# neeek2303/EMOPortraits

Hardware: AMD Instinct MI355X
Metric: reenactment frames/sec @512x512, 1-src->N-driver (higher is better)
Workload: dtype f32

## Files before the change

emoportraits_amd/csrc/conv_igemm_f16x2_ct2.h:

```cpp
#pragma once
#include "conv_igemm_bf16x3.h"
#include "conv_split_pair_common.h"

#ifndef EMO_CT2_RES_EARLY
#define EMO_CT2_RES_EARLY 0
#endif

template <int TR, int TW, bool UPS>
struct ConvCfgS2 : ConvCfgS<TR, TW, UPS, 2> {
  using Base = ConvCfgS<TR, TW, UPS, 2>;
  static_assert(Base::NWB == 2 && Base::EPI_IN_W, "two whole weight stages in LDS; the epilogue transposes through one of them");
  static constexpr int OFF_BIAS2_F = Base::OFF_EPI_F;
  static constexpr int OFF_STAT2_F = OFF_BIAS2_F + Base::BM;
  static constexpr int LDS_BYTES = (OFF_STAT2_F + 2 * Base::WGP * Base::BM) * 4;
  static_assert(LDS_BYTES <= 160 * 1024, "LDS");
  static_assert(Base::PBUF * 16 >= 8 * 1024, "the dead weight pieces of an item's last step are dumped into a patch buffer");
};

template <int TR, int TW, bool UPS>
__global__ __launch_bounds__(256) __attribute__((amdgpu_waves_per_eu(1, 1)))
void conv_igemm_bf16x3_ct2_kernel(const ConvArgs a) {
  using Cfg = ConvCfgS2<TR, TW, UPS>;
  using opx8 = halfx8;
  constexpr int SPLIT = 2, NPL = 2, NPROD = 3;
  constexpr int BM = Cfg::BM, TM = Cfg::TM, TP = Cfg::TP, WGP = Cfg::WGP, KC = Cfg::KC;
  constexpr int PR = Cfg::PR, NQ = Cfg::NQ, NQ1 = Cfg::NQ1, SUB = Cfg::SUB, CHS = Cfg::CHS, QPG = Cfg::QPG;
  constexpr int NHQ = Cfg::NHQ, TWS = Cfg::TWS, WPLANE = Cfg::WPLANE, WROW = Cfg::WROW, PPL = Cfg::PPL, PBUF = Cfg::PBUF;

  extern __shared__ __attribute__((aligned(16))) float smem[];

  const int tid = threadIdx.x;
  const int lane = tid & 63;
  const int wave = __builtin_amdgcn_readfirstlane(tid >> 6);
  const int half = lane >> 5, l32 = lane & 31;
  const int wp = wave;
  const int p0 = wp * TP * 32;
  float sat_m = 0.0f;

  const int HW = a.H * a.W;
  const long DHW = (long)a.D * HW;
  const bool has_affine = a.scale != nullptr;
  const int epi_mode = __builtin_amdgcn_readfirstlane(a.res == nullptr ? 0 : (a.res_ups ? 2 : 1));
  const float in_scale = a.in_scale;
  const int padD = a.KD >> 1;
  constexpr float CLAMP_HI = 65504.0f;
  const float clamp_lo = a.relu_in ? 0.0f : -CLAMP_HI;
  const int nst = a.n_cchunks * a.KD;
  const int nptiles = a.tiles_x * a.tiles_y * a.tiles_z;

  const int q_u = tid % QPG;
  const int q_g = __builtin_amdgcn_readfirstlane(tid / QPG);
  const bool is_quad = q_u < PR * NQ;
  const int hq = q_u - PR * NQ;
  const bool is_halo = !is_quad && hq < NHQ;
  const int h_side = hq & 1;
  const int q_r = is_quad ? q_u / NQ : (is_halo ? hq >> 1 : 0);
  const int q_c = is_quad ? q_u - q_r * NQ : 0;
  int q_slb[4];
#pragma unroll
  for (int i = 0; i < 4; ++i) {
    const int dump = q_g * CHS + i * SUB + PR * NQ1 + (q_u & 3);
    const int own = is_quad ? q_g * CHS + i * SUB + q_r * NQ1 + q_c : q_g * CHS + h_side * SUB + q_r * NQ1 + NQ;
    q_slb[i] = ((is_quad || (is_halo && i == (h_side ? 0 : 3))) ? own : dump) * 16;
  }

  floatx16 acc_lo[2][TM][TP], acc_hi[2][TM][TP];

  const int q8 = a.n_work >> 3, r8 = a.n_work & 7;
  const int xcd = blockIdx.x & 7;
  const int n_mine = q8 + (xcd < r8 ? 1 : 0);
  const int l_base = xcd < r8 ? xcd * (q8 + 1) : r8 * (q8 + 1) + (xcd - r8) * q8;
  const int l_stride = (gridDim.x + 7) >> 3;
  int it_cotile = 0, it_n = 0, it_ptile = 0, it_x0 = 0, it_y0 = 0, it_z0 = 0;
  unsigned lq_off = 0;
  bool lq_ok = false;
  int lq_z0 = 0;
#define EMO_T_WPTR(c_, k_) (reinterpret_cast<const char*>(a.wpk) + (long)((c_) * nst + (k_)) * (3 * Cfg::WROW_BYTES))

  const int a_off = (half * BM + l32) * 16;
  EMO_P_DECLARE_B_OFF()

  const char* const lds_c = reinterpret_cast<const char*>(smem);
  char* const lds_w = reinterpret_cast<char*>(smem);
  opx8 fa_[2][NPL][TM], fb_[2][NPL][TP];
#define EMO_T_LOAD_FRAGS_PLANE(set_, pl_, wbase_, pbyte_, r_, s_)                                      \
  {                                                                                                   \
    _Pragma("unroll") for (int i = 0; i < TM; ++i)                                                    \
      fa_[set_][pl_][i] = *reinterpret_cast<const opx8*>(lds_c + a_off + ((wbase_) + (pl_) * WPLANE + (s_) * 2 * BM + i * 32) * 16); \
    _Pragma("unroll") for (int j = 0; j < TP; ++j)                                                    \
      fb_[set_][pl_][j] = *reinterpret_cast<const opx8*>(lds_c + (EMO_P_B_OFF(j, r_, s_) + (pbyte_)) + ((pl_) * PPL) * 16); \
  }

  float* const sct = smem + Cfg::OFF_SCT * 4;
  const unsigned smem_lds = (unsigned)(size_t)(__attribute__((address_space(3))) char*)reinterpret_cast<char*>(smem);
  const unsigned lane16 = (unsigned)lane * 16u;

  floatx4 qv[8];
  float q_lo, q_hi;
  int q_tix;
  floatx4 q_sc, q_sh;
  opx8 cv_h, cv_m;
  emo_intx4 xrs = emo_raw_buffer(a.x);
  unsigned usoff[8];
#pragma unroll
  for (int u = 0; u < 8; ++u) usoff[u] = (unsigned)__builtin_amdgcn_readfirstlane((int)((unsigned)u * (unsigned)DHW * 4u * (EMO_CT2_X_CONST ? 0u : 1u)));

  int n_ci0, n_zu;
  bool n_zv;
  int ld_stage, ld_cc, ld_kd;
#define EMO_T_SET_STAGE_VARS()                                                                        \
  {                                                                                                   \
    n_ci0 = ld_cc * KC;                                                                               \
    n_zu = lq_z0 + ld_kd - padD;                                                                      \
    n_zv = (unsigned)n_zu < (unsigned)a.D;                                                            \
  }
  unsigned q_vo;
#define EMO_T_ISSUE_BEGIN()                                                                           \
  {                                                                                                   \
    const int c0_ = n_ci0 + q_g * 8;                                                                  \
    const bool cv_ = c0_ < a.Cin;                                                                     \
    const int cs_ = cv_ ? c0_ : 0;                                                                    \
    const bool keep_ = lq_ok && cv_ && n_zv;                                                          \
    q_lo = keep_ ? clamp_lo : 0.0f;                                                                   \
    q_hi = keep_ ? CLAMP_HI : 0.0f;                                                                   \
    q_vo = lq_off + (EMO_CT2_X_CONST ? 0u : ((unsigned)cs_ * (unsigned)DHW + (unsigned)((n_zv ? n_zu : 0) * HW)) * 4u);   \
    q_tix = (has_affine ? cs_ : (cs_ & (Cfg::SCT - 1))) >> 2;                                         \
  }
#define EMO_T_ISSUE_LOADS(u0_, u1_)                                                                   \
  { _Pragma("unroll") for (int u = (u0_); u < (u1_); u += 2) emo_bload4x2_pinned(xrs, q_vo, usoff[u], usoff[u + 1], qv[u], qv[u + 1]); }
#define EMO_T_HALF_TABLE(hf_)                                                                         \
  {                                                                                                   \
    const floatx4* t4_ = reinterpret_cast<const floatx4*>(sct) + q_tix + (hf_);                       \
    q_sc = t4_[0]; q_sh = t4_[Cfg::SCT / 4];                                                          \
  }
#define EMO_T_TOUCH_QUAD() { _Pragma("unroll") for (int u = 0; u < 8; ++u) emo_touch4(qv[u]); }
#define EMO_T_CONV_HALF(pbyte_, i_, hf_)                                                              \
  {                                                                                                   \
    float t_[4];                                                                                      \
    _Pragma("unroll") for (int k = 0; k < 4; ++k)                                                     \
      t_[k] = __fmaf_rn(qv[4 * (hf_) + k][i_], q_sc[k], q_sh[k]);                                     \
    sat_m = __builtin_fmaxf(__builtin_fmaxf(sat_m, __builtin_fabsf(t_[0])), __builtin_fabsf(t_[1])); \
    sat_m = __builtin_fmaxf(__builtin_fmaxf(sat_m, __builtin_fabsf(t_[2])), __builtin_fabsf(t_[3])); \
    _Pragma("unroll") for (int k = 0; k < 4; k += 2)                                                  \
      emo_split_f16x2_pair(__builtin_amdgcn_fmed3f(t_[k], q_lo, q_hi), __builtin_amdgcn_fmed3f(t_[k + 1], q_lo, q_hi), \
                           cv_h, cv_m, 4 * (hf_) + k);                                                \
    if ((hf_) == 1) {                                                                                 \
      char* d_ = lds_w + (q_slb[i_] + (pbyte_));                                                      \
      *reinterpret_cast<opx8*>(d_) = cv_h;                                                            \
      *reinterpret_cast<opx8*>(d_ + PPL * 16) = cv_m;                                                 \
    }                                                                                                 \
  }
#define EMO_T_WSRC(p_) (EMO_CT2_W_CONST ? reinterpret_cast<const char*>(a.wpk) : (p_))
#define EMO_T_DMA_PIECE(ptr_, wb_, k_)                                                                \
  {                                                                                                   \
    const int row_ = (k_) / 3, j_ = wave + 4 * ((k_) % 3);                                            \
    emo_dma16_pinned_s(EMO_T_WSRC((ptr_) + (row_ * Cfg::WROW_BYTES + j_ * 1024)), lane16,             \
                       smem_lds + (unsigned)((Cfg::OFF_W + (wb_) * Cfg::WSTAGE) * 16 + row_ * Cfg::WROW_BYTES + j_ * 1024)); \
  }

  constexpr int PA3[3] = {1, 0, 0}, PB3[3] = {0, 1, 0};
  constexpr int NTE = Cfg::SCT / 256;
  float te_sc[NTE], te_sh[NTE], te_b = 0.0f;

  bool chained_in = false;
  int pp = 0;
  for (int idx8 = blockIdx.x >> 3; idx8 < n_mine; idx8 += l_stride) {
#if EMO_S_TIMING
  unsigned long long tstamp[12];
  for (int k = 0; k < 12; ++k) tstamp[k] = 0;
#endif
  EMO_S_STAMP(0)
  EMO_P_DECODE(it_, l_base + idx8)
  int nx_cotile = 0, nx_n = 0, nx_ptile = 0, nx_x0 = 0, nx_y0 = 0, nx_z0 = 0;
  bool chain_out = false, nxq_ok = false;
  unsigned nxq_off = 0;
  if (EMO_S_CHAIN && idx8 + l_stride < n_mine) {
    EMO_P_DECODE(nx_, l_base + idx8 + l_stride)
    chain_out = nx_n == it_n && nst >= 2;
    EMO_P_CURSOR_OF(nx_, nxq_ok, nxq_off)
  }
  (void)nx_ptile;
#pragma unroll
  for (int st_ = 0; st_ < 2; ++st_)
#pragma unroll
    for (int pl = 0; pl < NPL; ++pl) {
#pragma unroll
      for (int i = 0; i < TM; ++i) asm volatile("" : "=v"(fa_[st_][pl][i]));
#pragma unroll
      for (int j = 0; j < TP; ++j) asm volatile("" : "=v"(fb_[st_][pl][j]));
    }
  asm volatile("" : "=v"(cv_h));
  asm volatile("" : "=v"(cv_m));
  if (EMO_S_CHAIN && chained_in) {
    xrs = emo_raw_buffer(a.x + (long)it_n * a.Cin * DHW);
    if (tid < 2 * BM) {
      const int t2_ = tid & (BM - 1);
      smem[(tid < BM ? Cfg::OFF_BIAS_F : Cfg::OFF_BIAS2_F) + (t2_ >> 5) * 32 + (t2_ & 3) * 8 + ((t2_ & 31) >> 2)] = te_b;
    }
    const char* const w1_ = EMO_T_WPTR(it_cotile + 1, 0);
    EMO_T_DMA_PIECE(w1_, 1, 0)
    EMO_T_DMA_PIECE(w1_, 1, 1)
    EMO_P_BARRIER(2);
  } else {
#pragma unroll
    for (int u = 0; u < 8; ++u) asm volatile("" : "=v"(qv[u]));
    xrs = emo_raw_buffer(a.x + (long)it_n * a.Cin * DHW);
    EMO_P_CURSOR_OF(it_, lq_ok, lq_off)
    lq_z0 = it_z0;
#pragma unroll
    for (int k = 0; k < NTE; ++k) {
      const int c = tid + 256 * k;
      const bool real = has_affine && c < a.Cin;
      te_sc[k] = real ? a.scale[(long)it_n * a.Cin + c] : 1.0f;
      te_sh[k] = real ? a.shift[(long)it_n * a.Cin + c] : 0.0f;
    }
    if (tid < 2 * BM && a.bias != nullptr) {
      const int co_ = it_cotile * BM + tid;
      te_b = a.bias[co_ < a.Cout ? co_ : a.Cout - 1];
    }
    {
      const char* const w0_ = EMO_T_WPTR(it_cotile, 0);
#pragma unroll
      for (int k = 0; k < 9; ++k) EMO_T_DMA_PIECE(w0_, 0, k)
    }
    ld_stage = 0; ld_cc = 0; ld_kd = 0;
    EMO_T_SET_STAGE_VARS()
    EMO_T_ISSUE_BEGIN()
    EMO_T_ISSUE_LOADS(0, 8)
#pragma unroll
    for (int k = 0; k < NTE; ++k) {
      const int c = tid + 256 * k;
      if (c < min(a.Cin, Cfg::SCT)) {
        sct[c] = te_sc[k] * in_scale;
        sct[Cfg::SCT + c] = te_sh[k] * in_scale;
      }
    }
    if (tid < 2 * BM) {
      const int t2_ = tid & (BM - 1);
      smem[(tid < BM ? Cfg::OFF_BIAS_F : Cfg::OFF_BIAS2_F) + (t2_ >> 5) * 32 + (t2_ & 3) * 8 + ((t2_ & 31) >> 2)] = te_b;
    }
    EMO_P_WAIT(0);
    EMO_T_TOUCH_QUAD()
    __syncthreads();
#pragma unroll
    for (int i = 0; i < 4; ++i) {
      EMO_T_HALF_TABLE(0)
      EMO_T_CONV_HALF(Cfg::OFF_P * 16, i, 0)
      EMO_T_HALF_TABLE(1)
      EMO_T_CONV_HALF(Cfg::OFF_P * 16, i, 1)
    }
    if (nst > 1) {
      ++ld_stage;
      if (++ld_kd == a.KD) { ld_kd = 0; ++ld_cc; }
    }
    EMO_T_SET_STAGE_VARS()
    EMO_T_ISSUE_BEGIN()
    EMO_T_ISSUE_LOADS(0, 8)
    EMO_T_HALF_TABLE(0)
    {
      const char* const w1_ = EMO_T_WPTR(it_cotile + 1, 0);
      EMO_T_DMA_PIECE(w1_, 1, 0)
      EMO_T_DMA_PIECE(w1_, 1, 1)
    }
    EMO_P_BARRIER(0);
    EMO_T_TOUCH_QUAD()
    pp = 0;
  }

  floatx4 rv_first[8];
#if EMO_CT2_RES_EARLY
  if (epi_mode == 1) conv_epilogue_fast_issue<TW, TP, BM, 1, 0, true>(a, rv_first, it_n, it_cotile, it_x0, it_y0, it_z0, wp, lane);
  else if (epi_mode == 2) conv_epilogue_fast_issue<TW, TP, BM, 2, 0, true>(a, rv_first, it_n, it_cotile, it_x0, it_y0, it_z0, wp, lane);
#endif
  EMO_S_STAMP(1)
#pragma unroll
  for (int c = 0; c < 2; ++c)
#pragma unroll
    for (int i = 0; i < TM; ++i)
#pragma unroll
      for (int j = 0; j < TP; ++j)
#pragma unroll
        for (int r = 0; r < 16; ++r) { acc_lo[c][i][j][r] = 0.0f; acc_hi[c][i][j][r] = 0.0f; }
  {
    const int pb0_ = (Cfg::OFF_P + pp * PBUF) * 16;
#pragma unroll
    for (int pl = 0; pl < NPL; ++pl) EMO_T_LOAD_FRAGS_PLANE(0, pl, Cfg::OFF_W, pb0_, 0, 0)
  }
  for (int cg = 0; cg < nst; ++cg) {
    const int pcur_b = (Cfg::OFF_P + pp * PBUF) * 16, pnxt_b = (Cfg::OFF_P + (pp ^ 1) * PBUF) * 16;
    const bool last_ = cg + 1 >= nst;
#pragma unroll
    for (int h = 0; h < 2; ++h) {
      const int c1_ = h == 0 ? it_cotile + 1 : (last_ && chain_out ? nx_cotile : it_cotile);
      const int k1_ = h == 0 ? cg : (last_ ? (chain_out ? 0 : nst - 1) : cg + 1);
      const int c2_ = (last_ && chain_out ? nx_cotile : it_cotile) + h;
      const int k2_ = last_ ? (chain_out ? 0 : nst - 1) : cg + 1;
      const char* const dma_ptr = EMO_T_WPTR(c1_, k1_);
      const char* const dma_ptr2 = EMO_T_WPTR(c2_, k2_);
      if (EMO_CONV_SETPRIO) __builtin_amdgcn_s_setprio(1);
#pragma unroll
      for (int gs = 0; gs < 9; ++gs) {
        const int r = gs / 3, s = gs % 3;
        const int fcur = (h * 9 + gs) & 1, fnxt = fcur ^ 1;
        (void)r; (void)s;
        if (gs == 8) { EMO_P_BARRIER(0); }
        if (gs == 8 && h == 1) EMO_T_TOUCH_QUAD()
        if (gs == 0 && h == 1) {
          const bool sw_ = chain_out && cg + 2 == nst;
          const int tgt_ = (chain_out && cg + 2 > nst) ? 1 : ((cg + 2) < nst ? cg + 2 : nst - 1);
          lq_ok = sw_ ? nxq_ok : lq_ok;
          lq_off = sw_ ? nxq_off : lq_off;
          lq_z0 = sw_ ? nx_z0 : lq_z0;
          const int adv_ = (!sw_ && tgt_ != ld_stage) ? 1 : 0;
          int kd_ = ld_kd + adv_, cc_ = ld_cc;
          if (kd_ == a.KD) { kd_ = 0; ++cc_; }
          ld_stage = sw_ ? 0 : ld_stage + adv_;
          ld_cc = sw_ ? 0 : cc_;
          ld_kd = sw_ ? 0 : kd_;
          EMO_T_SET_STAGE_VARS()
          EMO_T_ISSUE_BEGIN()
        }
        __builtin_amdgcn_sched_barrier(0);
        {
          const int rn = gs < 8 ? (gs + 1) / 3 : 0, sn = gs < 8 ? (gs + 1) % 3 : 0;
          const int wbn = Cfg::OFF_W + (gs < 8 ? h : h ^ 1) * Cfg::WSTAGE + rn * WROW;
          const int pbn = (gs == 8 && h == 1) ? pnxt_b : pcur_b;
#pragma unroll
          for (int pl = 0; pl < NPL + 1; ++pl) {
            if (pl < NPL) EMO_T_LOAD_FRAGS_PLANE(fnxt, pl, wbn, pbn, rn, sn)
            if (gs == 8 && pl < 2) {
              const int j_ = wave + 4 * pl;
              const unsigned dst_ = smem_lds + ((h == 1 && last_) ? (unsigned)(pcur_b + j_ * 1024)
                                                                   : (unsigned)((Cfg::OFF_W + h * Cfg::WSTAGE) * 16 + j_ * 1024));
              emo_dma16_pinned_s(EMO_T_WSRC(dma_ptr2 + j_ * 1024), lane16, dst_);
            }
            if (gs < 4 && pl == 0) EMO_T_DMA_PIECE(dma_ptr, h ^ 1, 2 + gs)
            if (h == 1 && gs < 4 && pl == 1) EMO_T_ISSUE_LOADS(2 * gs, 2 * gs + 2)
            if (gs == 4) EMO_T_DMA_PIECE(dma_ptr, h ^ 1, 6 + pl)
          }
        }
        if (h == 0 && gs < 8) {
          EMO_T_CONV_HALF(pnxt_b, gs >> 1, gs & 1)
          if (gs < 7) { EMO_T_HALF_TABLE((gs + 1) & 1) }
        }
        if (h == 1 && gs == 7) { EMO_T_HALF_TABLE(0) }
#pragma unroll
        for (int p = 0; p < NPROD; ++p) {
          const int pa = PA3[p], pb = PB3[p];
#pragma unroll
          for (int i = 0; i < TM; ++i)
#pragma unroll
            for (int j = 0; j < TP; ++j) {
              floatx16& acc_ = (pa == 0 && pb == 0) ? acc_lo[h][i][j] : acc_hi[h][i][j];
              acc_ = __builtin_amdgcn_mfma_f32_32x32x16_f16(fb_[fcur][pb][j], fa_[fcur][pa][i], acc_, 0, 0, 0);
            }
        }
        if (EMO_S_PIN) {
#pragma unroll
          for (int k = 0; k < 4 * NPL; ++k) {
            __builtin_amdgcn_sched_group_barrier(0x008, 1, 0);
            __builtin_amdgcn_sched_group_barrier(0x100, 1, 0);
            __builtin_amdgcn_sched_group_barrier(0x002, 5, 0);
          }
#pragma unroll
          for (int k = 4 * NPL; k < 4 * NPROD; ++k) {
            __builtin_amdgcn_sched_group_barrier(0x008, 1, 0);
            __builtin_amdgcn_sched_group_barrier(0x002, 6, 0);
            __builtin_amdgcn_sched_group_barrier(0x200, 1, 0);
          }
        }
        __builtin_amdgcn_sched_barrier(0);
      }
      if (EMO_CONV_SETPRIO) __builtin_amdgcn_s_setprio(0);
    }
    pp ^= 1;
  }
  EMO_S_STAMP(2)
  {
    float* const scratch = smem + (Cfg::OFF_W + Cfg::WSTAGE) * 4 + wave * Cfg::EPI_WAVE;
    const int ep_n = it_n, ep_cotile = it_cotile, ep_ptile = it_ptile, ep_x0 = it_x0, ep_y0 = it_y0, ep_z0 = it_z0;
    EMO_P_WAIT(0);
    EMO_S_STAMP(5)
    __syncthreads();
    EMO_S_STAMP(6)
    EMO_S_STAMP(7)
    if (EMO_S_CHAIN && chain_out && tid < 2 * BM && a.bias != nullptr) {
      const int co_ = nx_cotile * BM + tid;
      te_b = a.bias[co_ < a.Cout ? co_ : a.Cout - 1];
    }
#define EMO_T_EPI_FAST(RES_)                                                                                                      \
    {                                                                                                                              \
      floatx4 (&rv_)[8] = rv_first;                                                                                                \
      floatx4 rvn_[8];                                                                                                             \
      if (!EMO_CT2_RES_EARLY) conv_epilogue_fast_issue<TW, TP, BM, RES_, 0, true>(a, rv_, ep_n, ep_cotile, ep_x0, ep_y0, ep_z0, wp, lane); \
      conv_epilogue_fast_issue<TW, TP, BM, RES_, 0, true>(a, rvn_, ep_n, ep_cotile + 1, ep_x0, ep_y0, ep_z0, wp, lane);            \
      conv_epilogue_fast_finish<TW, TM, TP, WGP, BM, SPLIT, Cfg::EPI_ROWF, RES_, true, true>(                                      \
          a, acc_lo[0], acc_hi[0], rv_, scratch, smem + Cfg::OFF_BIAS_F, smem + Cfg::OFF_STAT_F, ep_n, ep_cotile, ep_ptile, ep_x0,  \
          ep_y0, ep_z0, wp, half, l32, lane, tid EMO_S_TSTAMP_ARG);                                                                \
      EMO_S_STAMP(10)                                                                                                              \
      conv_epilogue_fast_finish<TW, TM, TP, WGP, BM, SPLIT, Cfg::EPI_ROWF, RES_, true, true>(                                      \
          a, acc_lo[1], acc_hi[1], rvn_, scratch, smem + Cfg::OFF_BIAS2_F, smem + Cfg::OFF_STAT2_F, ep_n, ep_cotile + 1, ep_ptile,  \
          ep_x0, ep_y0, ep_z0, wp, half, l32, lane, tid EMO_S_TSTAMP_ARG);                                                         \
    }
    if (epi_mode == 1) EMO_T_EPI_FAST(1)
    else if (epi_mode == 2) EMO_T_EPI_FAST(2)
    else EMO_T_EPI_FAST(0)
#if EMO_S_TIMING
    tstamp[8] = tstamp[10];
#endif
#undef EMO_T_EPI_FAST
  }
  if (a.sat_flag != nullptr && sat_m > 65504.0f) *a.sat_flag = 1;
#if EMO_S_TIMING
  EMO_S_STAMP(3)
  asm volatile("s_waitcnt vmcnt(0)" ::: "memory");
  EMO_S_STAMP(4)
  {
    const int ep_L_ = l_base + idx8;
    if (tid == 0 && ep_L_ < EMO_S_TLOG_N) {
      unsigned long long* t_ = emo_s_tlog + (long)ep_L_ * EMO_S_TLOG_W;
#pragma unroll
      for (int k = 0; k < 12; ++k) t_[k] = tstamp[k];
      t_[12] = (unsigned long long)__builtin_amdgcn_s_getreg((31 << 11) | 4);
      t_[13] = (unsigned long long)__builtin_amdgcn_s_getreg((31 << 11) | 20);
      t_[14] = (unsigned long long)blockIdx.x;
    }
  }
#endif
  __syncthreads();
  EMO_P_COMBINE_STATS(Cfg::OFF_STAT_F, Cfg::OFF_STAT2_F, true)
  chained_in = chain_out;
  }
#undef EMO_T_WPTR
#undef EMO_T_LOAD_FRAGS_PLANE
#undef EMO_T_SET_STAGE_VARS
#undef EMO_T_ISSUE_BEGIN
#undef EMO_T_ISSUE_LOADS
#undef EMO_T_HALF_TABLE
#undef EMO_T_TOUCH_QUAD
#undef EMO_T_CONV_HALF
#undef EMO_T_DMA_PIECE
#undef EMO_T_WSRC
}

template <int TR, int TW, bool UPS>
int conv_f16x2_ct2_launch(ConvArgs a, hipStream_t s, int* rest_cot0) {
  using Cfg = ConvCfgS2<TR, TW, UPS>;
  *rest_cot0 = 0;
  const char* const e_on = getenv("EMO_CONV_CT2");
  if ((e_on && atoi(e_on) == 0) || !conv_pair_form<Cfg, TR, TW>(a)) return EMO_OK;
  const int pairs = (a.Cout / Cfg::BM) / 2;
  int grid = 0;
  if (!conv_pair_fill<TR, TW>(a, pairs, Cfg::KC, &grid)) return EMO_OK;
  auto kern = conv_igemm_bf16x3_ct2_kernel<TR, TW, UPS>;
  const int rc = emo_raise_dynamic_lds(kern);
  if (rc != EMO_OK) return rc;
  *rest_cot0 = 2 * pairs;
  return emo_launch(kern, dim3((unsigned)grid), dim3(256), (size_t)Cfg::LDS_BYTES, s, a);
}
```

Baseline: 423.7.

## Interleave both cout tiles per tap with a row-slotted weight ring in LDS

Reorganizes the paired-cout-tile conv kernel so each tap computes both output-channel tiles back to back, sharing one patch fragment load instead of sweeping tile 0 then tile 1. Weights now sit in three row slots holding both tiles, streamed tap by tap through a rolling DMA schedule spread across the 9 taps. The epilogue scratch is relocated behind the surviving taps plus an extra per-wave area. This is meant to halve patch fragment LDS reads and smooth the DMA and barrier cadence. In exchange it adds register copies of the B fragments per step, a more intricate prefetch hazard schedule, and a larger LDS footprint.

```diff
diff --git a/emoportraits_amd/csrc/conv_igemm_f16x2_ct2.h b/emoportraits_amd/csrc/conv_igemm_f16x2_ct2.h
--- a/emoportraits_amd/csrc/conv_igemm_f16x2_ct2.h
+++ b/emoportraits_amd/csrc/conv_igemm_f16x2_ct2.h
@@ -9,12 +9,15 @@
 template <int TR, int TW, bool UPS>
 struct ConvCfgS2 : ConvCfgS<TR, TW, UPS, 2> {
   using Base = ConvCfgS<TR, TW, UPS, 2>;
-  static_assert(Base::NWB == 2 && Base::EPI_IN_W, "two whole weight stages in LDS; the epilogue transposes through one of them");
+  static_assert(Base::NWB == 2 && Base::EPI_IN_W, "two whole weight stages in LDS (here: three row slots of both tiles)");
   static constexpr int OFF_BIAS2_F = Base::OFF_EPI_F;
   static constexpr int OFF_STAT2_F = OFF_BIAS2_F + Base::BM;
-  static constexpr int LDS_BYTES = (OFF_STAT2_F + 2 * Base::WGP * Base::BM) * 4;
+  static constexpr int OFF_EPI_W = Base::OFF_W + 3 * Base::WROW + Base::WPLANE + 2 * 2 * Base::BM;
+  static_assert(OFF_EPI_W * 4 + 3 * Base::EPI_WAVE <= (Base::OFF_W + 6 * Base::WROW) * 4, "three waves' scratch behind the surviving taps");
+  static constexpr int OFF_EPI3_F = OFF_STAT2_F + 2 * Base::WGP * Base::BM;
+  static_assert(OFF_EPI3_F % 4 == 0, "16-byte rows");
+  static constexpr int LDS_BYTES = (OFF_EPI3_F + Base::EPI_WAVE) * 4;
   static_assert(LDS_BYTES <= 160 * 1024, "LDS");
-  static_assert(Base::PBUF * 16 >= 8 * 1024, "the dead weight pieces of an item's last step are dumped into a patch buffer");
 };
 
 template <int TR, int TW, bool UPS>
@@ -83,12 +86,18 @@
   const char* const lds_c = reinterpret_cast<const char*>(smem);
   char* const lds_w = reinterpret_cast<char*>(smem);
   opx8 fa_[2][NPL][TM], fb_[2][NPL][TP];
-#define EMO_T_LOAD_FRAGS_PLANE(set_, pl_, wbase_, pbyte_, r_, s_)                                      \
-  {                                                                                                   \
+#define EMO_T_WSLOT(r_, c_) (Cfg::OFF_W + (2 * (r_) + (c_)) * WROW)
+#define EMO_T_LOAD_WFRAGS(c_, r_, s_)                                                                 \
+  {                                                                                                   \
+    _Pragma("unroll") for (int pl = 0; pl < NPL; ++pl)                                                \
     _Pragma("unroll") for (int i = 0; i < TM; ++i)                                                    \
-      fa_[set_][pl_][i] = *reinterpret_cast<const opx8*>(lds_c + a_off + ((wbase_) + (pl_) * WPLANE + (s_) * 2 * BM + i * 32) * 16); \
+      fa_[c_][pl][i] = *reinterpret_cast<const opx8*>(lds_c + a_off + (EMO_T_WSLOT(r_, c_) + pl * WPLANE + (s_) * 2 * BM + i * 32) * 16); \
+  }
+#define EMO_T_LOAD_PFRAGS(set_, pbyte_, r_, s_)                                                       \
+  {                                                                                                   \
+    _Pragma("unroll") for (int pl = 0; pl < NPL; ++pl)                                                \
     _Pragma("unroll") for (int j = 0; j < TP; ++j)                                                    \
-      fb_[set_][pl_][j] = *reinterpret_cast<const opx8*>(lds_c + (EMO_P_B_OFF(j, r_, s_) + (pbyte_)) + ((pl_) * PPL) * 16); \
+      fb_[set_][pl][j] = *reinterpret_cast<const opx8*>(lds_c + (EMO_P_B_OFF(j, r_, s_) + (pbyte_)) + (pl * PPL) * 16); \
   }
 
   float* const sct = smem + Cfg::OFF_SCT * 4;
@@ -151,11 +160,16 @@
     }                                                                                                 \
   }
 #define EMO_T_WSRC(p_) (EMO_CT2_W_CONST ? reinterpret_cast<const char*>(a.wpk) : (p_))
-#define EMO_T_DMA_PIECE(ptr_, wb_, k_)                                                                \
-  {                                                                                                   \
-    const int row_ = (k_) / 3, j_ = wave + 4 * ((k_) % 3);                                            \
-    emo_dma16_pinned_s(EMO_T_WSRC((ptr_) + (row_ * Cfg::WROW_BYTES + j_ * 1024)), lane16,             \
-                       smem_lds + (unsigned)((Cfg::OFF_W + (wb_) * Cfg::WSTAGE) * 16 + row_ * Cfg::WROW_BYTES + j_ * 1024)); \
+  const int w_poff = __builtin_amdgcn_readfirstlane(((wave >> 1) * WPLANE + (wave & 1) * BM) * 16);
+  const unsigned lds_wv = smem_lds + (unsigned)w_poff;
+  unsigned w_voff[9];
+#pragma unroll
+  for (int g = 0; g < 9; ++g)
+    w_voff[g] = lane16 + (EMO_CT2_W_CONST ? 0u : (unsigned)((g / 3) * Cfg::WROW_BYTES + (g % 3) * 2 * BM * 16 + w_poff));
+#define EMO_T_DMA_TAP(p0_, p1_, g_)                                                                   \
+  {                                                                                                   \
+    emo_dma16_pinned_s(EMO_T_WSRC(p0_), w_voff[g_], lds_wv + (unsigned)(EMO_T_WSLOT((g_) / 3, 0) * 16 + ((g_) % 3) * 2 * BM * 16)); \
+    emo_dma16_pinned_s(EMO_T_WSRC(p1_), w_voff[g_], lds_wv + (unsigned)(EMO_T_WSLOT((g_) / 3, 1) * 16 + ((g_) % 3) * 2 * BM * 16)); \
   }
 
   constexpr int PA3[3] = {1, 0, 0}, PB3[3] = {0, 1, 0};
@@ -197,10 +211,6 @@
       const int t2_ = tid & (BM - 1);
       smem[(tid < BM ? Cfg::OFF_BIAS_F : Cfg::OFF_BIAS2_F) + (t2_ >> 5) * 32 + (t2_ & 3) * 8 + ((t2_ & 31) >> 2)] = te_b;
     }
-    const char* const w1_ = EMO_T_WPTR(it_cotile + 1, 0);
-    EMO_T_DMA_PIECE(w1_, 1, 0)
-    EMO_T_DMA_PIECE(w1_, 1, 1)
-    EMO_P_BARRIER(2);
   } else {
 #pragma unroll
     for (int u = 0; u < 8; ++u) asm volatile("" : "=v"(qv[u]));
@@ -218,11 +228,10 @@
       const int co_ = it_cotile * BM + tid;
       te_b = a.bias[co_ < a.Cout ? co_ : a.Cout - 1];
     }
-    {
-      const char* const w0_ = EMO_T_WPTR(it_cotile, 0);
-#pragma unroll
-      for (int k = 0; k < 9; ++k) EMO_T_DMA_PIECE(w0_, 0, k)
-    }
+    const char* const w0_ = EMO_T_WPTR(it_cotile, 0);
+    const char* const w1_ = EMO_T_WPTR(it_cotile + 1, 0);
+#pragma unroll
+    for (int g = 0; g < 5; ++g) EMO_T_DMA_TAP(w0_, w1_, g)
     ld_stage = 0; ld_cc = 0; ld_kd = 0;
     EMO_T_SET_STAGE_VARS()
     EMO_T_ISSUE_BEGIN()
@@ -257,11 +266,6 @@
     EMO_T_ISSUE_BEGIN()
     EMO_T_ISSUE_LOADS(0, 8)
     EMO_T_HALF_TABLE(0)
-    {
-      const char* const w1_ = EMO_T_WPTR(it_cotile + 1, 0);
-      EMO_T_DMA_PIECE(w1_, 1, 0)
-      EMO_T_DMA_PIECE(w1_, 1, 1)
-    }
     EMO_P_BARRIER(0);
     EMO_T_TOUCH_QUAD()
     pp = 0;
@@ -283,29 +287,29 @@
         for (int r = 0; r < 16; ++r) { acc_lo[c][i][j][r] = 0.0f; acc_hi[c][i][j][r] = 0.0f; }
   {
     const int pb0_ = (Cfg::OFF_P + pp * PBUF) * 16;
-#pragma unroll
-    for (int pl = 0; pl < NPL; ++pl) EMO_T_LOAD_FRAGS_PLANE(0, pl, Cfg::OFF_W, pb0_, 0, 0)
-  }
+    EMO_T_LOAD_WFRAGS(0, 0, 0)
+    EMO_T_LOAD_PFRAGS(0, pb0_, 0, 0)
+  }
+  const long w_tile = (long)nst * (3 * Cfg::WROW_BYTES);
+  const char* cur_p0 = EMO_T_WPTR(it_cotile, 0);
+  const char* const end_p0 = chain_out ? EMO_T_WPTR(nx_cotile, 0) : EMO_T_WPTR(it_cotile, nst - 1);
   for (int cg = 0; cg < nst; ++cg) {
     const int pcur_b = (Cfg::OFF_P + pp * PBUF) * 16, pnxt_b = (Cfg::OFF_P + (pp ^ 1) * PBUF) * 16;
     const bool last_ = cg + 1 >= nst;
-#pragma unroll
-    for (int h = 0; h < 2; ++h) {
-      const int c1_ = h == 0 ? it_cotile + 1 : (last_ && chain_out ? nx_cotile : it_cotile);
-      const int k1_ = h == 0 ? cg : (last_ ? (chain_out ? 0 : nst - 1) : cg + 1);
-      const int c2_ = (last_ && chain_out ? nx_cotile : it_cotile) + h;
-      const int k2_ = last_ ? (chain_out ? 0 : nst - 1) : cg + 1;
-      const char* const dma_ptr = EMO_T_WPTR(c1_, k1_);
-      const char* const dma_ptr2 = EMO_T_WPTR(c2_, k2_);
-      if (EMO_CONV_SETPRIO) __builtin_amdgcn_s_setprio(1);
-#pragma unroll
-      for (int gs = 0; gs < 9; ++gs) {
-        const int r = gs / 3, s = gs % 3;
-        const int fcur = (h * 9 + gs) & 1, fnxt = fcur ^ 1;
-        (void)r; (void)s;
-        if (gs == 8) { EMO_P_BARRIER(0); }
-        if (gs == 8 && h == 1) EMO_T_TOUCH_QUAD()
-        if (gs == 0 && h == 1) {
+    const char* const cur_p1 = cur_p0 + w_tile;
+    const char* const dma_p0 = last_ ? end_p0 : cur_p0 + 3 * Cfg::WROW_BYTES;
+    const char* const dma_p1 = dma_p0 + w_tile;
+    if (EMO_CONV_SETPRIO) __builtin_amdgcn_s_setprio(1);
+#pragma unroll
+    for (int gs = 0; gs < 9; ++gs) {
+      const int r = gs / 3, s = gs % 3;
+      const int fcur = gs & 1, fnxt = fcur ^ 1;
+      (void)r; (void)s;
+#pragma unroll
+      for (int h = 0; h < 2; ++h) {
+        if (h == 1 && (gs == 3 || gs == 8)) { EMO_P_BARRIER(0); }
+        if (h == 1 && gs == 8) EMO_T_TOUCH_QUAD()
+        if (h == 0 && gs == 4) {
           const bool sw_ = chain_out && cg + 2 == nst;
           const int tgt_ = (chain_out && cg + 2 > nst) ? 1 : ((cg + 2) < nst ? cg + 2 : nst - 1);
           lq_ok = sw_ ? nxq_ok : lq_ok;
@@ -321,27 +325,26 @@
           EMO_T_ISSUE_BEGIN()
         }
         __builtin_amdgcn_sched_barrier(0);
-        {
+        if (h == 0) {
+          EMO_T_LOAD_WFRAGS(1, r, s)
+          if (gs == 0) { EMO_T_DMA_TAP(cur_p0, cur_p1, 5) EMO_T_DMA_TAP(cur_p0, cur_p1, 6) }
+          if (gs == 1) EMO_T_DMA_TAP(cur_p0, cur_p1, 8)
+          if (gs == 4) EMO_T_ISSUE_LOADS(0, 4)
+          if (gs == 5) EMO_T_DMA_TAP(dma_p0, dma_p1, 1)
+          if (gs == 6) EMO_T_DMA_TAP(dma_p0, dma_p1, 3)
+        } else {
           const int rn = gs < 8 ? (gs + 1) / 3 : 0, sn = gs < 8 ? (gs + 1) % 3 : 0;
-          const int wbn = Cfg::OFF_W + (gs < 8 ? h : h ^ 1) * Cfg::WSTAGE + rn * WROW;
-          const int pbn = (gs == 8 && h == 1) ? pnxt_b : pcur_b;
-#pragma unroll
-          for (int pl = 0; pl < NPL + 1; ++pl) {
-            if (pl < NPL) EMO_T_LOAD_FRAGS_PLANE(fnxt, pl, wbn, pbn, rn, sn)
-            if (gs == 8 && pl < 2) {
-              const int j_ = wave + 4 * pl;
-              const unsigned dst_ = smem_lds + ((h == 1 && last_) ? (unsigned)(pcur_b + j_ * 1024)
-                                                                   : (unsigned)((Cfg::OFF_W + h * Cfg::WSTAGE) * 16 + j_ * 1024));
-              emo_dma16_pinned_s(EMO_T_WSRC(dma_ptr2 + j_ * 1024), lane16, dst_);
-            }
-            if (gs < 4 && pl == 0) EMO_T_DMA_PIECE(dma_ptr, h ^ 1, 2 + gs)
-            if (h == 1 && gs < 4 && pl == 1) EMO_T_ISSUE_LOADS(2 * gs, 2 * gs + 2)
-            if (gs == 4) EMO_T_DMA_PIECE(dma_ptr, h ^ 1, 6 + pl)
-          }
+          EMO_T_LOAD_WFRAGS(0, rn, sn)
+          EMO_T_LOAD_PFRAGS(fnxt, gs == 8 ? pnxt_b : pcur_b, rn, sn)
+          if (gs == 0) EMO_T_DMA_TAP(cur_p0, cur_p1, 7)
+          if (gs == 3) EMO_T_DMA_TAP(dma_p0, dma_p1, 0)
+          if (gs == 4) EMO_T_ISSUE_LOADS(4, 8)
+          if (gs == 5) EMO_T_DMA_TAP(dma_p0, dma_p1, 2)
+          if (gs == 8) EMO_T_DMA_TAP(dma_p0, dma_p1, 4)
         }
-        if (h == 0 && gs < 8) {
-          EMO_T_CONV_HALF(pnxt_b, gs >> 1, gs & 1)
-          if (gs < 7) { EMO_T_HALF_TABLE((gs + 1) & 1) }
+        if (gs < 4) {
+          EMO_T_CONV_HALF(pnxt_b, gs, h)
+          if (2 * gs + h < 7) { EMO_T_HALF_TABLE(h ^ 1) }
         }
         if (h == 1 && gs == 7) { EMO_T_HALF_TABLE(0) }
 #pragma unroll
@@ -352,18 +355,19 @@
 #pragma unroll
             for (int j = 0; j < TP; ++j) {
               floatx16& acc_ = (pa == 0 && pb == 0) ? acc_lo[h][i][j] : acc_hi[h][i][j];
-              acc_ = __builtin_amdgcn_mfma_f32_32x32x16_f16(fb_[fcur][pb][j], fa_[fcur][pa][i], acc_, 0, 0, 0);
+              acc_ = __builtin_amdgcn_mfma_f32_32x32x16_f16(fb_[fcur][pb][j], fa_[h][pa][i], acc_, 0, 0, 0);
             }
         }
         if (EMO_S_PIN) {
-#pragma unroll
-          for (int k = 0; k < 4 * NPL; ++k) {
+          const int NRD = TM * NPL * (1 + h);
+#pragma unroll
+          for (int k = 0; k < NRD; ++k) {
             __builtin_amdgcn_sched_group_barrier(0x008, 1, 0);
             __builtin_amdgcn_sched_group_barrier(0x100, 1, 0);
             __builtin_amdgcn_sched_group_barrier(0x002, 5, 0);
           }
 #pragma unroll
-          for (int k = 4 * NPL; k < 4 * NPROD; ++k) {
+          for (int k = NRD; k < 4 * NPROD; ++k) {
             __builtin_amdgcn_sched_group_barrier(0x008, 1, 0);
             __builtin_amdgcn_sched_group_barrier(0x002, 6, 0);
             __builtin_amdgcn_sched_group_barrier(0x200, 1, 0);
@@ -371,13 +375,18 @@
         }
         __builtin_amdgcn_sched_barrier(0);
       }
-      if (EMO_CONV_SETPRIO) __builtin_amdgcn_s_setprio(0);
-    }
+    }
+    if (EMO_CONV_SETPRIO) __builtin_amdgcn_s_setprio(0);
+#pragma unroll
+    for (int pl = 0; pl < NPL; ++pl)
+#pragma unroll
+      for (int j = 0; j < TP; ++j) fb_[0][pl][j] = fb_[1][pl][j];
+    cur_p0 = dma_p0;
     pp ^= 1;
   }
   EMO_S_STAMP(2)
   {
-    float* const scratch = smem + (Cfg::OFF_W + Cfg::WSTAGE) * 4 + wave * Cfg::EPI_WAVE;
+    float* const scratch = smem + (wave < 3 ? Cfg::OFF_EPI_W * 4 + wave * Cfg::EPI_WAVE : Cfg::OFF_EPI3_F);
     const int ep_n = it_n, ep_cotile = it_cotile, ep_ptile = it_ptile, ep_x0 = it_x0, ep_y0 = it_y0, ep_z0 = it_z0;
     EMO_P_WAIT(0);
     EMO_S_STAMP(5)
@@ -432,14 +441,16 @@
   chained_in = chain_out;
   }
 #undef EMO_T_WPTR
-#undef EMO_T_LOAD_FRAGS_PLANE
+#undef EMO_T_WSLOT
+#undef EMO_T_LOAD_WFRAGS
+#undef EMO_T_LOAD_PFRAGS
 #undef EMO_T_SET_STAGE_VARS
 #undef EMO_T_ISSUE_BEGIN
 #undef EMO_T_ISSUE_LOADS
 #undef EMO_T_HALF_TABLE
 #undef EMO_T_TOUCH_QUAD
 #undef EMO_T_CONV_HALF
-#undef EMO_T_DMA_PIECE
+#undef EMO_T_DMA_TAP
 #undef EMO_T_WSRC
 }
 
```

Measured after the change: 427.7 (median of 6 runs). Within noise of the previous version (+0.9%).
